# TencentYoutuResearch/NeRF-Loc

Measured on AMD Instinct MI355X. Metric: rendered rays/sec (4096 rays×128 samples, 256-wide MLP) at 1/2/4/8 MI355X, higher is better.
Workload: dtype f16mx (neural-point kernel, conv_out and feat_mlp.0: fp16 hi.hi + two MX-FP6 cross terms, 1.5 MFMA-equivalents per product; every other GEMM 3-term split-bf16 or split-fp16; fp32 accumulate; meets 1e-4)

## Files before the change

### nerf_loc_amd/csrc/knn.hip

```cpp
#include "common.h"

namespace {

constexpr int GRID_BITS = 6;
constexpr int GRID_N = 1 << GRID_BITS;
constexpr int GRID_CELLS = GRID_N * GRID_N * GRID_N;

__device__ __forceinline__ unsigned part1by2(unsigned x) {
  x &= 0x3ffu;
  x = (x | (x << 16)) & 0x030000FFu;
  x = (x | (x << 8)) & 0x0300F00Fu;
  x = (x | (x << 4)) & 0x030C30C3u;
  x = (x | (x << 2)) & 0x09249249u;
  return x;
}
__device__ __forceinline__ unsigned morton3(unsigned x, unsigned y, unsigned z) {
  return part1by2(x) | (part1by2(y) << 1) | (part1by2(z) << 2);
}

__global__ void knn_bbox_kernel(const float* __restrict__ xyz, int M, NlGridParams* gp) {
  __shared__ float smin[3][256], smax[3][256];
  float mn[3] = {3.4e38f, 3.4e38f, 3.4e38f}, mx[3] = {-3.4e38f, -3.4e38f, -3.4e38f};
  for (int i = threadIdx.x; i < M; i += blockDim.x) {
#pragma unroll
    for (int d = 0; d < 3; ++d) {
      float v = xyz[3 * (size_t)i + d];
      mn[d] = fminf(mn[d], v);
      mx[d] = fmaxf(mx[d], v);
    }
  }
#pragma unroll
  for (int d = 0; d < 3; ++d) { smin[d][threadIdx.x] = mn[d]; smax[d][threadIdx.x] = mx[d]; }
  __syncthreads();
  for (int s = blockDim.x / 2; s > 0; s >>= 1) {
    if ((int)threadIdx.x < s) {
#pragma unroll
      for (int d = 0; d < 3; ++d) {
        smin[d][threadIdx.x] = fminf(smin[d][threadIdx.x], smin[d][threadIdx.x + s]);
        smax[d][threadIdx.x] = fmaxf(smax[d][threadIdx.x], smax[d][threadIdx.x + s]);
      }
    }
    __syncthreads();
  }
  if (threadIdx.x == 0) {
    float ext = 0.f;
    for (int d = 0; d < 3; ++d) ext = fmaxf(ext, smax[d][0] - smin[d][0]);
    float cell = ext > 0.f ? ext / (float)GRID_N : 1.f;
    cell *= 1.0001f;
    gp->cell = cell;
    gp->inv_cell = 1.f / cell;
    for (int d = 0; d < 3; ++d) {
      gp->origin[d] = smin[d][0];
      gp->bmax[d] = smax[d][0];
      gp->dims[d] = GRID_N;
    }
    gp->ncells = GRID_CELLS;
  }
}

__device__ __forceinline__ int cell_coord(float v, float origin, float inv_cell) {
  int c = (int)floorf((v - origin) * inv_cell);
  return c < 0 ? 0 : (c >= GRID_N ? GRID_N - 1 : c);
}

__global__ void knn_count_kernel(const float* __restrict__ xyz, int M, const NlGridParams* __restrict__ gp,
                                 int* __restrict__ counts, int* __restrict__ cell_of) {
  int i = blockIdx.x * blockDim.x + threadIdx.x;
  if (i >= M) return;
  int cx = cell_coord(xyz[3 * (size_t)i + 0], gp->origin[0], gp->inv_cell);
  int cy = cell_coord(xyz[3 * (size_t)i + 1], gp->origin[1], gp->inv_cell);
  int cz = cell_coord(xyz[3 * (size_t)i + 2], gp->origin[2], gp->inv_cell);
  int cid = (int)morton3(cx, cy, cz);
  cell_of[i] = cid;
  atomicAdd(&counts[cid], 1);
}

__global__ void knn_scan_kernel(const int* __restrict__ counts, int* __restrict__ starts, int* __restrict__ cursor) {
  __shared__ int part[1024];
  const int n = GRID_CELLS;
  const int per = n / 1024;
  const int b = threadIdx.x * per;
  int s = 0;
  for (int i = b; i < b + per; ++i) s += counts[i];
  part[threadIdx.x] = s;
  __syncthreads();
  for (int o = 1; o < 1024; o <<= 1) {
    int v = (int)threadIdx.x >= o ? part[threadIdx.x - o] : 0;
    __syncthreads();
    part[threadIdx.x] += v;
    __syncthreads();
  }
  int run = threadIdx.x ? part[threadIdx.x - 1] : 0;
  for (int i = b; i < b + per; ++i) {
    starts[i] = run;
    cursor[i] = run;
    run += counts[i];
  }
  if (threadIdx.x == 1023) starts[n] = part[1023];
}

__global__ void knn_scatter_kernel(const float* __restrict__ xyz, int M, const int* __restrict__ cell_of,
                                   int* __restrict__ cursor, float4* __restrict__ sorted) {
  int i = blockIdx.x * blockDim.x + threadIdx.x;
  if (i >= M) return;
  int pos = atomicAdd(&cursor[cell_of[i]], 1);
  sorted[pos] = make_float4(xyz[3 * (size_t)i], xyz[3 * (size_t)i + 1], xyz[3 * (size_t)i + 2], __int_as_float(i));
}

typedef unsigned long long u64;

template <int CTRL, int ROWMASK>
__device__ __forceinline__ unsigned dpp_umin(unsigned v) {
  const unsigned t = (unsigned)__builtin_amdgcn_update_dpp((int)0xffffffffu, (int)v, CTRL, ROWMASK, 0xf, false);
  return t < v ? t : v;
}
__device__ __forceinline__ unsigned wave_umin(unsigned v) {
  v = dpp_umin<0x111, 0xf>(v);
  v = dpp_umin<0x112, 0xf>(v);
  v = dpp_umin<0x114, 0xf>(v);
  v = dpp_umin<0x118, 0xf>(v);
  v = dpp_umin<0x142, 0xa>(v);
  v = dpp_umin<0x143, 0xc>(v);
  return (unsigned)__builtin_amdgcn_readlane((int)v, 63);
}

template <int CTRL, int ROWMASK>
__device__ __forceinline__ unsigned dpp_umax(unsigned v) {
  const unsigned t = (unsigned)__builtin_amdgcn_update_dpp(0, (int)v, CTRL, ROWMASK, 0xf, false);
  return t > v ? t : v;
}
__device__ __forceinline__ unsigned wave_umax(unsigned v) {
  v = dpp_umax<0x111, 0xf>(v); v = dpp_umax<0x112, 0xf>(v); v = dpp_umax<0x114, 0xf>(v); v = dpp_umax<0x118, 0xf>(v);
  v = dpp_umax<0x142, 0xa>(v); v = dpp_umax<0x143, 0xc>(v);
  return (unsigned)__builtin_amdgcn_readlane((int)v, 63);
}

template <int K>
struct BestK {
  unsigned d, i, p;
  unsigned td, ti;
  __device__ __forceinline__ void clear() { d = i = td = ti = 0xffffffffu; p = 0; }
  __device__ __forceinline__ bool full() const { return ti != 0xffffffffu; }
  __device__ __forceinline__ void insert(unsigned nd, unsigned ni, unsigned np) {
    const unsigned pd = (unsigned)__builtin_amdgcn_update_dpp(0, (int)d, 0x111, 0xf, 0xf, false);
    const unsigned pi = (unsigned)__builtin_amdgcn_update_dpp(0, (int)i, 0x111, 0xf, 0xf, false);
    const unsigned pp = (unsigned)__builtin_amdgcn_update_dpp(0, (int)p, 0x111, 0xf, 0xf, false);
    const bool lt_me = nd < d || (nd == d && ni < i);
    const bool lt_prev = nd < pd || (nd == pd && ni < pi);
    d = lt_me ? (lt_prev ? pd : nd) : d;
    i = lt_me ? (lt_prev ? pi : ni) : i;
    p = lt_me ? (lt_prev ? pp : np) : p;
    td = (unsigned)__builtin_amdgcn_readlane((int)d, K - 1);
    ti = (unsigned)__builtin_amdgcn_readlane((int)i, K - 1);
  }
  __device__ __forceinline__ unsigned idx_at(int k) const { return (unsigned)__builtin_amdgcn_readlane((int)i, k); }
};

#ifdef KNN_STATS
__device__ unsigned long long knn_stats[16];
#define KNN_CNT(i, v) do { if (__lane_id() == 0) atomicAdd(&knn_stats[i], (unsigned long long)(v)); } while (0)
#else
#define KNN_CNT(i, v)
#endif
template <int K>
__device__ __forceinline__ void select_into(BestK<K>& best, unsigned kd, unsigned ki, unsigned kp) {
  while (true) {
    const bool cont = kd < best.td || (kd == best.td && ki < best.ti);
    if (__ballot(cont) == 0ull) break;
    KNN_CNT(2, 1);
    const unsigned dmin = wave_umin(cont ? kd : 0xffffffffu);
    const bool tie = cont && kd == dmin;
    const u64 tm = __ballot(tie);
    unsigned imin;
    int src = __builtin_ctzll(tm);
    if (__popcll(tm) == 1) imin = (unsigned)__builtin_amdgcn_readlane((int)ki, src);
    else {
      imin = wave_umin(tie ? ki : 0xffffffffu);
      src = __builtin_ctzll(__ballot(tie && ki == imin));
    }
    best.insert(dmin, imin, (unsigned)__builtin_amdgcn_readlane((int)kp, src));
    if (tie && ki == imin) { kd = 0xffffffffu; ki = 0xffffffffu; }
  }
}

struct QueryCtx {
  float qx, qy, qz, org0, org1, org2, cell, slack;
};

__device__ __forceinline__ float node_mindist2(const QueryCtx& c, unsigned cx, unsigned cy, unsigned cz, int L) {
  const float cl = c.cell * (float)(1 << L);
  const float x0 = c.org0 + (float)cx * cl, y0 = c.org1 + (float)cy * cl, z0 = c.org2 + (float)cz * cl;
  const float dx = fmaxf(fmaxf(x0 - c.qx, c.qx - (x0 + cl)) - c.slack, 0.f);
  const float dy = fmaxf(fmaxf(y0 - c.qy, c.qy - (y0 + cl)) - c.slack, 0.f);
  const float dz = fmaxf(fmaxf(z0 - c.qz, c.qz - (z0 + cl)) - c.slack, 0.f);
  return dx * dx + dy * dy + dz * dz;
}

template <int K, bool DEDUPE>
__device__ __forceinline__ void candidate(const QueryCtx& c, const float4* __restrict__ sorted, bool valid, int pos, const BestK<K>& best,
                                          unsigned& kd, unsigned& ki, bool dedupe_now = true, unsigned ubits = 0xffffffffu) {
  kd = 0xffffffffu; ki = 0xffffffffu;
  if (valid) {
    const float4 p = sorted[pos];
    const float ddx = c.qx - p.x, ddy = c.qy - p.y, ddz = c.qz - p.z;
    float d = __fmul_rn(ddx, ddx);
    d = __fadd_rn(d, __fmul_rn(ddy, ddy));
    d = __fadd_rn(d, __fmul_rn(ddz, ddz));
    kd = __float_as_uint(d);
    ki = (unsigned)__float_as_int(p.w);
    if (kd > ubits) { kd = 0xffffffffu; ki = 0xffffffffu; }
    if (DEDUPE && dedupe_now) {
      bool dup = false;
#pragma unroll
      for (int k = 0; k < K; ++k) dup |= (ki == best.idx_at(k));
      if (dup) { kd = 0xffffffffu; ki = 0xffffffffu; }
    }
  }
}

template <int K, bool DEDUPE, class Sink>
__device__ __forceinline__ void scan_range(const QueryCtx& c, const float4* __restrict__ sorted, int rs, int len, int lane, BestK<K>& best, Sink&& sink,
                                           bool dedupe_now = true, unsigned ubits = 0xffffffffu) {
  for (int base = 0; base < len; base += 64) {
    KNN_CNT(3, 1);
    unsigned kd, ki;
    candidate<K, DEDUPE>(c, sorted, base + lane < len, rs + base + lane, best, kd, ki, dedupe_now, ubits);
    sink(kd, ki, (unsigned)(rs + base + lane));
  }
}

constexpr int FRONT_CAP = 128;
constexpr int LEAF_CAP = 128;
constexpr int LEAF_COUNT_MAX = 8;

template <int K, int SPW>
__global__ __launch_bounds__(256) void knn_wave_kernel(const float* __restrict__ q, int N, const NlGridParams* __restrict__ gpp,
                                                       const int* __restrict__ starts, const float4* __restrict__ sorted,
                                                       int Kout, int* __restrict__ idx_out, float* __restrict__ d2_out) {
  __shared__ unsigned s_front[4][2][FRONT_CAP], s_fxyz[4][2][FRONT_CAP];
  __shared__ int s_leaf_s[4][LEAF_CAP], s_leaf_l[4][LEAF_CAP];
  __shared__ u64 s_ckey[4][64];
  __shared__ unsigned s_cpos[4][64];
  const int lane = threadIdx.x & 63, wv = threadIdx.x >> 6;
  const int n0 = __builtin_amdgcn_readfirstlane((nl_xcd_block() * 4 + wv) * SPW);
  QueryCtx c;
  c.org0 = gpp->origin[0]; c.org1 = gpp->origin[1]; c.org2 = gpp->origin[2];
  c.cell = gpp->cell; c.slack = 1e-3f * c.cell;
  const float inv_cell = gpp->inv_cell;
  bool prev_full = false;
  unsigned ppos = 0;
  bool pkeep = false;
  u64* const ckey = s_ckey[wv];
  unsigned* const cpos = s_cpos[wv];

  for (int sq = 0; sq < SPW; ++sq) {
  const int n = n0 + sq;
  if (n >= N) return;
  c.qx = q[3 * (size_t)n]; c.qy = q[3 * (size_t)n + 1]; c.qz = q[3 * (size_t)n + 2];

  BestK<K> best;
  best.clear();
  float U;
  const bool dedupe_now = !prev_full;
  bool deferred = prev_full;
  int ncand = 0;
  auto lds_list_handover = [&]() __attribute__((always_inline)) {
    __builtin_amdgcn_fence(__ATOMIC_RELEASE, "wavefront");
    __builtin_amdgcn_wave_barrier();
    __builtin_amdgcn_fence(__ATOMIC_ACQUIRE, "wavefront");
  };
  auto pour = [&]() __attribute__((always_inline)) {
    unsigned kd = 0xffffffffu, ki = 0xffffffffu, kp = 0;
    lds_list_handover();
    if (lane < ncand) { const u64 k = ckey[lane]; kd = (unsigned)(k >> 32); ki = (unsigned)k; kp = cpos[lane]; }
    select_into<K>(best, kd, ki, kp);
    ncand = 0;
    deferred = false;
  };
  const u64 lt_mask = (1ull << lane) - 1ull;
  auto sink = [&](unsigned kd, unsigned ki, unsigned kp) __attribute__((always_inline)) {
    if (!deferred) { select_into<K>(best, kd, ki, kp); return; }
    const bool v = ki != 0xffffffffu;
    const u64 mv = __ballot(v);
    if (mv == 0ull) return;
    const int cn = __popcll(mv);
    if (ncand + cn > 64) { pour(); select_into<K>(best, kd, ki, kp); return; }
    if (v) { const int pos = ncand + __popcll(mv & lt_mask); ckey[pos] = ((u64)kd << 32) | (u64)ki; cpos[pos] = kp; }
    ncand += cn;
  };
  if (!prev_full) {
    unsigned m = 0, mx = 0, my = 0, mz = 0;
    int L = GRID_BITS;
    while (L > 0) {
      unsigned key = 0xffffffffu;
      if (lane < 8) {
        const unsigned mc = (m << 3) | (unsigned)lane;
        const int sh = 3 * (L - 1);
        const int cnt = starts[(mc + 1) << sh] - starts[mc << sh];
        if (cnt >= K)
          key = (__float_as_uint(node_mindist2(c, 2 * mx + (lane & 1), 2 * my + ((lane >> 1) & 1), 2 * mz + ((lane >> 2) & 1), L - 1)) & ~7u) | (unsigned)lane;
      }
      key = wave_umin(key);
      if (key == 0xffffffffu) break;
      const unsigned ch = key & 7u;
      m = (m << 3) | ch;
      mx = 2 * mx + (ch & 1); my = 2 * my + ((ch >> 1) & 1); mz = 2 * mz + ((ch >> 2) & 1);
      --L;
    }
    const int rs0 = starts[m << (3 * L)], len0 = starts[(m + 1) << (3 * L)] - rs0;
    scan_range<K, false>(c, sorted, rs0, len0, lane, best, sink);
    U = best.full() ? __uint_as_float(best.td) : 3.4e38f;
  } else {
    float dprev = 0.f;
    if (pkeep) {
      const float4 pt = sorted[ppos];
      const float ddx = c.qx - pt.x, ddy = c.qy - pt.y, ddz = c.qz - pt.z;
      dprev = __fadd_rn(__fadd_rn(__fmul_rn(ddx, ddx), __fmul_rn(ddy, ddy)), __fmul_rn(ddz, ddz));
    }
    U = __uint_as_float(wave_umax(__float_as_uint(dprev)));
  }

  unsigned* front = s_front[wv][0];
  unsigned* nextf = s_front[wv][1];
  unsigned* fxyz = s_fxyz[wv][0];
  unsigned* nextx = s_fxyz[wv][1];
  int* leaf_s = s_leaf_s[wv];
  int* leaf_l = s_leaf_l[wv];
  int nfront = 1, nleaf = 0;
  int Lstart = GRID_BITS;
  if (U < 3.0e38f) {
    const float r = sqrtf(U * 1.000001f) + c.slack;
    const int lo0 = min(max((int)floorf((c.qx - r - c.org0) * inv_cell) - 1, 0), GRID_N - 1), hi0 = min(max((int)floorf((c.qx + r - c.org0) * inv_cell) + 1, 0), GRID_N - 1);
    const int lo1 = min(max((int)floorf((c.qy - r - c.org1) * inv_cell) - 1, 0), GRID_N - 1), hi1 = min(max((int)floorf((c.qy + r - c.org1) * inv_cell) + 1, 0), GRID_N - 1);
    const int lo2 = min(max((int)floorf((c.qz - r - c.org2) * inv_cell) - 1, 0), GRID_N - 1), hi2 = min(max((int)floorf((c.qz + r - c.org2) * inv_cell) + 1, 0), GRID_N - 1);
    int Ls = 1;
    while (Ls < GRID_BITS && (((hi0 >> Ls) - (lo0 >> Ls)) > 1 || ((hi1 >> Ls) - (lo1 >> Ls)) > 1 || ((hi2 >> Ls) - (lo2 >> Ls)) > 1)) ++Ls;
    Ls = __builtin_amdgcn_readfirstlane(Ls);
    if (Ls < GRID_BITS) {
      Lstart = Ls;
      const unsigned nx = (unsigned)(lo0 >> Ls) + (lane & 1), ny = (unsigned)(lo1 >> Ls) + ((lane >> 1) & 1), nz = (unsigned)(lo2 >> Ls) + ((lane >> 2) & 1);
      const bool ok = lane < 8 && nx <= (unsigned)(hi0 >> Ls) && ny <= (unsigned)(hi1 >> Ls) && nz <= (unsigned)(hi2 >> Ls);
      const u64 mk = __ballot(ok);
      if (ok) { const int pos = __popcll(mk & lt_mask); front[pos] = morton3(nx, ny, nz); fxyz[pos] = nx | (ny << 10) | (nz << 20); }
      nfront = __popcll(mk);
    }
  }
  if (Lstart == GRID_BITS && lane == 0) { front[0] = 0u; fxyz[0] = 0u; }
  KNN_CNT(4, Lstart); KNN_CNT(5, prev_full ? 0 : 1); KNN_CNT(6 + Lstart, 1);

  auto flush_leaves = [&]() {
    constexpr int SL = LEAF_COUNT_MAX;
    for (int b = 0; b < nleaf; b += 64 / SL) {
      KNN_CNT(1, 1);
      const int e = b + lane / SL;
      const bool ok = e < nleaf;
      const int rs = ok ? leaf_s[e] : 0, ln = ok ? leaf_l[e] : 0;
      unsigned kd, ki;
      candidate<K, true>(c, sorted, (lane % SL) < ln, rs + (lane % SL), best, kd, ki, dedupe_now, __float_as_uint(U));
      sink(kd, ki, (unsigned)(rs + (lane % SL)));
    }
    nleaf = 0;
    if (best.full()) U = fminf(U, __uint_as_float(best.td));
  };

  for (int L = Lstart; L > 0; --L) {
    int nnext = 0;
    const int sh = 3 * (L - 1);
    for (int base = 0; base < nfront; base += 8) {
      KNN_CNT(0, 1);
      const int ni = base + (lane >> 3);
      bool keep = false, leaf = false;
      unsigned mc = 0, cxyz = 0;
      int rs = 0, cnt = 0;
      if (ni < nfront) {
        mc = (front[ni] << 3) | (unsigned)(lane & 7);
        const unsigned pxyz = fxyz[ni];
        const unsigned cx = 2 * (pxyz & 1023u) + (lane & 1), cy = 2 * ((pxyz >> 10) & 1023u) + ((lane >> 1) & 1), cz = 2 * (pxyz >> 20) + ((lane >> 2) & 1);
        cxyz = cx | (cy << 10) | (cz << 20);
        rs = starts[mc << sh];
        cnt = starts[(mc + 1) << sh] - rs;
        keep = cnt > 0 && node_mindist2(c, cx, cy, cz, L - 1) <= U * 1.000001f;
        leaf = keep && (L - 1 == 0 || cnt <= LEAF_COUNT_MAX);
      }
      const bool inner = keep && !leaf;
      const u64 mi = __ballot(inner);
      const int ci = __popcll(mi);
      const int room = FRONT_CAP - nnext;
      const int pi = __popcll(mi & lt_mask);
      const bool spill = inner && pi >= room;
      if (inner && !spill) { nextf[nnext + pi] = mc; nextx[nnext + pi] = cxyz; }
      nnext += ci < room ? ci : room;
      const bool lf = leaf || spill;
      u64 mbig = __ballot(lf && cnt > LEAF_COUNT_MAX);
      while (mbig) {
        const int src = __builtin_ctzll(mbig);
        mbig &= mbig - 1;
        scan_range<K, true>(c, sorted, __builtin_amdgcn_readlane(rs, src), __builtin_amdgcn_readlane(cnt, src), lane, best, sink, dedupe_now, __float_as_uint(U));
        if (best.full()) U = fminf(U, __uint_as_float(best.td));
      }
      const bool small = lf && cnt <= LEAF_COUNT_MAX;
      const u64 ml = __ballot(small);
      const int cl_ = __popcll(ml);
      if (nleaf + cl_ > LEAF_CAP) flush_leaves();
      if (small) { const int p = nleaf + __popcll(ml & lt_mask); leaf_s[p] = rs; leaf_l[p] = cnt; }
      nleaf += cl_;
      if (nleaf >= 32) flush_leaves();
    }
    unsigned* t = front; front = nextf; nextf = t;
    t = fxyz; fxyz = nextx; nextx = t;
    nfront = nnext;
    if (nfront == 0) break;
  }
  if (nleaf > 0) flush_leaves();

  if (deferred && ncand < K) pour();
  if (deferred) {
    lds_list_handover();
    const u64 mine = lane < ncand ? ckey[lane] : ~0ull;
    const unsigned mlo = (unsigned)mine, mhi = (unsigned)(mine >> 32);
    int rank = 0;
    for (int jj = 0; jj < ncand; ++jj) {
      const u64 kj = ((u64)(unsigned)__builtin_amdgcn_readlane((int)mhi, jj) << 32) | (u64)(unsigned)__builtin_amdgcn_readlane((int)mlo, jj);
      rank += kj < mine ? 1 : 0;
    }
    const bool win = lane < ncand && rank < K;
    if (win && rank < Kout) {
      idx_out[(size_t)n * Kout + rank] = (int)mlo;
      d2_out[(size_t)n * Kout + rank] = __uint_as_float(mhi);
    }
    prev_full = true;
    pkeep = win;
    ppos = cpos[lane];
  } else {
    if (lane < Kout && lane < K) {
      const unsigned bd = best.d, bi = best.i;
      const bool ok = bi != 0xffffffffu;
      idx_out[(size_t)n * Kout + lane] = ok ? (int)bi : 0;
      d2_out[(size_t)n * Kout + lane] = ok ? __uint_as_float(bd) : 0.f;
    }
    prev_full = best.full();
    pkeep = lane < K;
    ppos = best.p;
  }
  }
}

}

size_t nl_knn_grid_bytes(int64_t M) {
  size_t b = 0;
  b += nl_align_up(sizeof(NlGridParams), 256);
  b += nl_align_up(sizeof(int) * (GRID_CELLS + 1), 256);
  b += 2 * nl_align_up(sizeof(int) * GRID_CELLS, 256);
  b += nl_align_up(sizeof(int) * (size_t)(M > 0 ? M : 1), 256);
  b += nl_align_up(sizeof(float4) * (size_t)(M > 0 ? M : 1), 256);
  return b;
}

int nl_knn_grid_build(NlKnnGrid* g, void* mem, const float* xyz, int64_t M, hipStream_t st) {
  char* p = (char*)mem;
  g->params = (NlGridParams*)p; p += nl_align_up(sizeof(NlGridParams), 256);
  g->starts = (int*)p; p += nl_align_up(sizeof(int) * (GRID_CELLS + 1), 256);
  g->counts = (int*)p; p += nl_align_up(sizeof(int) * GRID_CELLS, 256);
  g->cursor = (int*)p; p += nl_align_up(sizeof(int) * GRID_CELLS, 256);
  g->cell_of = (int*)p; p += nl_align_up(sizeof(int) * (size_t)(M > 0 ? M : 1), 256);
  g->sorted = (float4*)p;
  g->M = (int)M;
  if (M <= 0) return NL_OK;
  NL_CHECK_HIP(hipMemsetAsync(g->counts, 0, sizeof(int) * GRID_CELLS, st));
  hipLaunchKernelGGL(knn_bbox_kernel, dim3(1), dim3(256), 0, st, xyz, (int)M, g->params);
  int nb = (int)nl_cdiv(M, 256);
  hipLaunchKernelGGL(knn_count_kernel, dim3(nb), dim3(256), 0, st, xyz, (int)M, g->params, g->counts, g->cell_of);
  hipLaunchKernelGGL(knn_scan_kernel, dim3(1), dim3(1024), 0, st, g->counts, g->starts, g->cursor);
  hipLaunchKernelGGL(knn_scatter_kernel, dim3(nb), dim3(256), 0, st, xyz, (int)M, g->cell_of, g->cursor, g->sorted);
  NL_LAUNCH_CHECK();
  return NL_OK;
}

int nl_knn_search(const NlKnnGrid* g, const float* xyz, int64_t N, int K, int* idx, float* d2, hipStream_t st) {
  if (N <= 0) return NL_OK;
  if (g->M <= 0) {
    NL_CHECK_HIP(hipMemsetAsync(idx, 0, sizeof(int) * (size_t)N * K, st));
    NL_CHECK_HIP(hipMemsetAsync(d2, 0, sizeof(float) * (size_t)N * K, st));
    return NL_OK;
  }
  if (K < 1 || K > 8) return NL_ERR_UNSUPPORTED;
  constexpr int spw_small = 4;
  const bool big = N >= (1 << 18);
  const int spw = big ? 16 : spw_small;
  dim3 grid(nl_xcd_grid(nl_cdiv(N, 4 * spw)));
#define NL_KNN(KK, SPW) hipLaunchKernelGGL((knn_wave_kernel<KK, SPW>), grid, dim3(256), 0, st, xyz, (int)N, g->params, g->starts, g->sorted, K, idx, d2)
  if (K == 1) { if (big) NL_KNN(1, 16); else NL_KNN(1, spw_small); }
  else { if (big) NL_KNN(8, 16); else NL_KNN(8, spw_small); }
#undef NL_KNN
  NL_LAUNCH_CHECK();
#ifdef KNN_STATS
  {
    unsigned long long h[16];
    hipStreamSynchronize(st);
    hipMemcpyFromSymbol(h, HIP_SYMBOL(knn_stats), sizeof(h));
    fprintf(stderr, "knn stats per query (N = %lld): frontier batches %.2f, leaf batches %.2f, selection iterations %.2f, range batches %.2f, start level %.2f, phase-1 %.3f; start-level histogram",
            (long long)N, (double)h[0] / N, (double)h[1] / N, (double)h[2] / N, (double)h[3] / N, (double)h[4] / N, (double)h[5] / N);
    for (int l = 0; l <= GRID_BITS; ++l) fprintf(stderr, " %d:%.3f", l, (double)h[6 + l] / N);
    fprintf(stderr, "\n");
    hipMemset(nullptr, 0, 0);
    unsigned long long z[16] = {0};
    hipMemcpyToSymbol(HIP_SYMBOL(knn_stats), z, sizeof(z));
  }
#endif
  return NL_OK;
}
```

### nerf_loc_amd/csrc/mvdec.h

```cpp
#pragma once
#include "common.h"
#include "mfma.h"

namespace nlmv {

struct Taps {
  int x0, y0;
  float nw, ne, sw, se;
  bool mw, me, mn, ms;
};

template <bool ALIGN, bool BORDER>
__device__ __forceinline__ Taps make_taps(float xn, float yn, int Wm, int Hm) {
  float ix, iy;
  if (ALIGN) {
    ix = (xn + 1.f) * ((float)(Wm - 1) / 2.f);
    iy = (yn + 1.f) * ((float)(Hm - 1) / 2.f);
  } else {
    ix = (xn + 1.f) * ((float)Wm / 2.f) - 0.5f;
    iy = (yn + 1.f) * ((float)Hm / 2.f) - 0.5f;
  }
  if (BORDER) {
    ix = fminf((float)(Wm - 1), fmaxf(ix, 0.f));
    iy = fminf((float)(Hm - 1), fmaxf(iy, 0.f));
  }
  float xw = floorf(ix), yn0 = floorf(iy);
  float w = ix - xw, e = 1.f - w, n = iy - yn0, s = 1.f - n;
  Taps t;
  t.nw = s * e; t.ne = s * w; t.sw = n * e; t.se = n * w;
  xw = fminf(fmaxf(xw, -2.f), (float)Wm + 1.f);
  yn0 = fminf(fmaxf(yn0, -2.f), (float)Hm + 1.f);
  t.x0 = (int)xw; t.y0 = (int)yn0;
  t.mw = t.x0 >= 0 && t.x0 < Wm;
  t.me = t.x0 + 1 >= 0 && t.x0 + 1 < Wm;
  t.mn = t.y0 >= 0 && t.y0 < Hm;
  t.ms = t.y0 + 1 >= 0 && t.y0 + 1 < Hm;
  return t;
}

__device__ __forceinline__ unsigned pack_taps(const Taps& t, int w, int h) {
  const int x0 = min(max(t.x0, 0), w - 1), x1 = min(max(t.x0 + 1, 0), w - 1);
  const int y0 = min(max(t.y0, 0), h - 1), y1 = min(max(t.y0 + 1, 0), h - 1);
  return (unsigned)(y0 * w + x0) | ((unsigned)(x1 - x0) << 30) | ((unsigned)(y1 - y0) << 31);
}
__device__ __forceinline__ void unpack_taps(unsigned pk, int w, int (&o)[4]) {
  const int base = (int)(pk & 0x3fffffffu), dx = (int)((pk >> 30) & 1u), dy = (pk >> 31) ? w : 0;
  o[0] = base; o[1] = base + dx; o[2] = base + dy; o[3] = base + dy + dx;
}


constexpr int DEC_STRIDE = 1024 + 32 + 1024 + 32 + 64 + 2;

__device__ __forceinline__ void decoder(const float* __restrict__ w, const float (&x)[32], float& o0, float& o1) {
  float h1[32], h2[32];
#pragma unroll
  for (int j = 0; j < 32; ++j) {
    float a = w[1024 + j];
#pragma unroll
    for (int i = 0; i < 32; ++i) a = fmaf(w[j * 32 + i], x[i], a);
    h1[j] = nl_elu(a);
  }
  const float* w2 = w + 1024 + 32;
#pragma unroll
  for (int j = 0; j < 32; ++j) {
    float a = w2[1024 + j];
#pragma unroll
    for (int i = 0; i < 32; ++i) a = fmaf(w2[j * 32 + i], h1[i], a);
    h2[j] = nl_elu(a);
  }
  const float* w4 = w2 + 1024 + 32;
  float a0 = w4[64], a1 = w4[65];
#pragma unroll
  for (int i = 0; i < 32; ++i) {
    a0 = fmaf(w4[i], h2[i], a0);
    a1 = fmaf(w4[32 + i], h2[i], a1);
  }
  o0 = a0;
  o1 = a1;
}


__device__ __forceinline__ bool project_neuray(const float* P, float X, float Y, float Z, int Wimg, int H, float& px, float& py, float& depth) {
  const float cx = fmaf(P[2], Z, fmaf(P[1], Y, P[0] * X)) + P[3];
  const float cy = fmaf(P[6], Z, fmaf(P[5], Y, P[4] * X)) + P[7];
  depth = fmaf(P[10], Z, fmaf(P[9], Y, P[8] * X)) + P[11];
  const bool bad = fabsf(depth) < 1e-4f;
  if (bad) depth = 1e-3f;
  px = cx / depth; py = cy / depth;
  const bool outside = (px < -0.5f) | (px >= (float)Wimg - 0.5f) | (py < -0.5f) | (py >= (float)H - 0.5f);
  return !bad && !outside;
}

__device__ __forceinline__ void sample_visf(const float* __restrict__ base, int h, int w, int Wimg, int H, float px, float py, bool valid, float (&x)[32]) {
  if (valid) {
    const float xn = px / (float)(Wimg - 1) * 2.f - 1.f;
    const float yn = py / (float)(H - 1) * 2.f - 1.f;
    const Taps t = make_taps<false, true>(xn, yn, w, h);
    const int xe = t.x0 + 1, ys = t.y0 + 1;
#pragma unroll
    for (int c4 = 0; c4 < 8; ++c4) {
      float4 a = make_float4(0, 0, 0, 0), b = a, c = a, d = a;
      if (t.mn && t.mw) a = *(const float4*)(base + ((size_t)t.y0 * w + t.x0) * 32 + c4 * 4);
      if (t.mn && t.me) b = *(const float4*)(base + ((size_t)t.y0 * w + xe) * 32 + c4 * 4);
      if (t.ms && t.mw) c = *(const float4*)(base + ((size_t)ys * w + t.x0) * 32 + c4 * 4);
      if (t.ms && t.me) d = *(const float4*)(base + ((size_t)ys * w + xe) * 32 + c4 * 4);
      x[c4 * 4 + 0] = a.x * t.nw + b.x * t.ne + c.x * t.sw + d.x * t.se;
      x[c4 * 4 + 1] = a.y * t.nw + b.y * t.ne + c.y * t.sw + d.y * t.se;
      x[c4 * 4 + 2] = a.z * t.nw + b.z * t.ne + c.z * t.sw + d.z * t.se;
      x[c4 * 4 + 3] = a.w * t.nw + b.w * t.ne + c.w * t.sw + d.w * t.se;
    }
  } else {
#pragma unroll
    for (int i = 0; i < 32; ++i) x[i] = 0.f;
  }
}

__device__ __forceinline__ void decode_all(const float* __restrict__ dw, const float (&x)[32], float& m0, float& m1, float& v0, float& v1, float& vs, float& aw) {
  float dummy;
  decoder(dw + 0 * DEC_STRIDE, x, m0, m1);
  decoder(dw + 1 * DEC_STRIDE, x, v0, v1);
  decoder(dw + 2 * DEC_STRIDE, x, aw, dummy);
  decoder(dw + 3 * DEC_STRIDE, x, vs, dummy);
  m0 = nl_softplus(m0); m1 = nl_softplus(m1);
  v0 = nl_softplus(v0) + 0.05f; v1 = nl_softplus(v1) + 0.05f;
  aw = nl_sigmoid(aw); vs = nl_sigmoid(vs);
}


constexpr int MVD_W1 = 0;
constexpr int MVD_W2 = 1024;
constexpr int MVD_F32 = 2048;
constexpr int MVD_NF32 = (128 + 128 + 256 + 8) / 4;
constexpr int MVD_F16 = MVD_F32 + MVD_NF32;
constexpr int MVD_T = MVD_F16 + 2048;
constexpr int MVD_PACK_UINT4 = MVD_T + 2048;
constexpr int MVD_LDS_UINT4 = 2048 + MVD_NF32;

template <bool X3>
__device__ __forceinline__ void mvd_load_lds(uint4* sw, const uint4* __restrict__ dpack, int tid, int nthreads) {
  for (int i = tid; i < 2048; i += nthreads) sw[i] = dpack[(X3 ? MVD_F16 : 0) + i];
  for (int i = tid; i < MVD_NF32; i += nthreads) sw[2048 + i] = dpack[MVD_F32 + i];
}

template <bool X3> struct MvdOps;
template <> struct MvdOps<true> {
  typedef nl_f16x8 v8;
  static __device__ __forceinline__ void split(const float (&v)[8], v8& hi, v8& lo) {
    nl_u32x4 h, l;
#pragma unroll
    for (int t = 0; t < 4; ++t) {
      unsigned hp, lp; float l0, l1;
      asm("v_cvt_pk_f16_f32 %0, %3, %4\n\tv_fma_mix_f32 %1, %0, -1.0, %3 op_sel_hi:[1,0,0]\n\tv_fma_mix_f32 %2, %0, -1.0, %4 op_sel:[1,0,0] op_sel_hi:[1,0,0]"
          : "=&v"(hp), "=&v"(l0), "=&v"(l1) : "v"(v[2 * t]), "v"(v[2 * t + 1]));
      asm("v_cvt_pk_f16_f32 %0, %1, %2" : "=v"(lp) : "v"(l0), "v"(l1));
      h[t] = hp; l[t] = lp;
    }
    hi = __builtin_bit_cast(v8, h); lo = __builtin_bit_cast(v8, l);
  }
  static __device__ __forceinline__ nl_f32x16 mfma(v8 a, v8 b, nl_f32x16 c) { return __builtin_amdgcn_mfma_f32_32x32x16_f16(a, b, c, 0, 0, 0); }
};
template <> struct MvdOps<false> {
  typedef nl_bf16x8 v8;
  static __device__ __forceinline__ void split(const float (&v)[8], v8& hi, v8& lo) {
#pragma unroll
    for (int t = 0; t < 8; ++t) hi[t] = (__bf16)v[t];
    lo = hi;
  }
  static __device__ __forceinline__ nl_f32x16 mfma(v8 a, v8 b, nl_f32x16 c) { return __builtin_amdgcn_mfma_f32_32x32x16_bf16(a, b, c, 0, 0, 0); }
};

__device__ __forceinline__ void mvd_elu2(float& a, float& b) { const nl_f32x2 e = nl_elu_fast2(nl_f32x2{a, b}); a = e[0]; b = e[1]; }

__device__ __forceinline__ void mvd_tap16(const float* __restrict__ base , int vh, int vw_, int Wimg, int H, float px, float py,
                                          bool valid, float (&x0)[8], float (&x1)[8]) {
  const float xn = px / (float)(Wimg - 1) * 2.f - 1.f;
  const float yn = py / (float)(H - 1) * 2.f - 1.f;
  const Taps t = make_taps<false, true>(xn, yn, vw_, vh);
  const size_t o00 = ((size_t)(t.mn ? t.y0 : 0) * vw_ + (t.mw ? t.x0 : 0)) * 32;
  const size_t o01 = ((size_t)(t.mn ? t.y0 : 0) * vw_ + (t.me ? t.x0 + 1 : 0)) * 32;
  const size_t o10 = ((size_t)(t.ms ? t.y0 + 1 : 0) * vw_ + (t.mw ? t.x0 : 0)) * 32;
  const size_t o11 = ((size_t)(t.ms ? t.y0 + 1 : 0) * vw_ + (t.me ? t.x0 + 1 : 0)) * 32;
  const float w00 = (valid && t.mn && t.mw) ? t.nw : 0.f, w01 = (valid && t.mn && t.me) ? t.ne : 0.f;
  const float w10 = (valid && t.ms && t.mw) ? t.sw : 0.f, w11 = (valid && t.ms && t.me) ? t.se : 0.f;
#pragma unroll
  for (int g = 0; g < 2; ++g) {
#pragma unroll
    for (int c4 = 0; c4 < 2; ++c4) {
      const int co = 16 * g + 4 * c4;
      const float4 a = *(const float4*)(base + o00 + co), b = *(const float4*)(base + o01 + co);
      const float4 c = *(const float4*)(base + o10 + co), d = *(const float4*)(base + o11 + co);
      float* dst = g ? x1 : x0;
      dst[4 * c4 + 0] = fmaf(d.x, w11, fmaf(c.x, w10, fmaf(b.x, w01, a.x * w00)));
      dst[4 * c4 + 1] = fmaf(d.y, w11, fmaf(c.y, w10, fmaf(b.y, w01, a.y * w00)));
      dst[4 * c4 + 2] = fmaf(d.z, w11, fmaf(c.z, w10, fmaf(b.z, w01, a.z * w00)));
      dst[4 * c4 + 3] = fmaf(d.w, w11, fmaf(c.w, w10, fmaf(b.w, w01, a.w * w00)));
    }
  }
}

template <bool X3>
__device__ __forceinline__ void mvd_decode_tile(const uint4* sw, int lane, const float (&x0)[8], const float (&x1)[8], float& m0, float& m1,
                                                float& v0, float& v1, float& vs, float& aw) {
  typedef MvdOps<X3> OP;
  typedef typename OP::v8 v8;
  const int hh = lane >> 5;
  const float* sf = reinterpret_cast<const float*>(sw + 2048);
  const float* b1 = sf, *b2 = sf + 128, *w4p = sf + 256, *b4 = sf + 512;
  v8 xh[2], xl[2];
  OP::split(x0, xh[0], xl[0]);
  OP::split(x1, xh[1], xl[1]);
  float o[4][2];
#pragma unroll
  for (int d = 0; d < 4; ++d) {
    nl_f32x16 acc;
#pragma unroll
    for (int g = 0; g < 4; ++g) {
      const float4 b = *(const float4*)(b1 + 32 * d + 8 * g + 4 * hh);
      acc[4 * g] = b.x; acc[4 * g + 1] = b.y; acc[4 * g + 2] = b.z; acc[4 * g + 3] = b.w;
    }
#pragma unroll
    for (int q = 0; q < 2; ++q) {
      const v8 ah = __builtin_bit_cast(v8, sw[MVD_W1 + (q * 4 + d) * 64 + lane]);
      if (X3) {
        const v8 al = __builtin_bit_cast(v8, sw[MVD_W1 + 512 + (q * 4 + d) * 64 + lane]);
        acc = OP::mfma(al, xh[q], acc);
        acc = OP::mfma(ah, xl[q], acc);
      }
      acc = OP::mfma(ah, xh[q], acc);
    }
    v8 gh[2], gl[2];
#pragma unroll
    for (int s = 0; s < 2; ++s) {
      float vv[8];
#pragma unroll
      for (int t = 0; t < 8; ++t) vv[t] = acc[8 * s + t];
#pragma unroll
      for (int t = 0; t < 8; t += 2) mvd_elu2(vv[t], vv[t + 1]);
      OP::split(vv, gh[s], gl[s]);
    }
    nl_f32x16 acc2;
#pragma unroll
    for (int g = 0; g < 4; ++g) {
      const float4 b = *(const float4*)(b2 + 32 * d + 8 * g + 4 * hh);
      acc2[4 * g] = b.x; acc2[4 * g + 1] = b.y; acc2[4 * g + 2] = b.z; acc2[4 * g + 3] = b.w;
    }
#pragma unroll
    for (int s = 0; s < 2; ++s) {
      const v8 ah = __builtin_bit_cast(v8, sw[MVD_W2 + (d * 2 + s) * 64 + lane]);
      if (X3) {
        const v8 al = __builtin_bit_cast(v8, sw[MVD_W2 + 512 + (d * 2 + s) * 64 + lane]);
        acc2 = OP::mfma(al, gh[s], acc2);
        acc2 = OP::mfma(ah, gl[s], acc2);
      }
      acc2 = OP::mfma(ah, gh[s], acc2);
    }
    float h2[16];
#pragma unroll
    for (int r = 0; r < 16; ++r) h2[r] = acc2[r];
#pragma unroll
    for (int r = 0; r < 16; r += 2) mvd_elu2(h2[r], h2[r + 1]);
#pragma unroll
    for (int u = 0; u < 2; ++u) {
      float p = 0.f;
      if (u == 0 || d < 2) {
        const float* w = w4p + ((d * 2 + u) * 2 + hh) * 16;
#pragma unroll
        for (int r4 = 0; r4 < 4; ++r4) {
          const float4 ww = *(const float4*)(w + 4 * r4);
          p = fmaf(ww.x, h2[4 * r4], p); p = fmaf(ww.y, h2[4 * r4 + 1], p);
          p = fmaf(ww.z, h2[4 * r4 + 2], p); p = fmaf(ww.w, h2[4 * r4 + 3], p);
        }
        p += __shfl_xor(p, 32, 64);
        p += b4[d * 2 + u];
      }
      o[d][u] = p;
    }
  }
  m0 = nl_softplus(o[0][0]); m1 = nl_softplus(o[0][1]);
  v0 = nl_softplus(o[1][0]) + 0.05f; v1 = nl_softplus(o[1][1]) + 0.05f;
  aw = nl_sigmoid(o[2][0]); vs = nl_sigmoid(o[3][0]);
}

}
```

Baseline: 580,100.

## Streamline KNN octree descent arithmetic and merge fp16 split asm

After: 584,900, median of 6. Within noise of the previous version (+0.8%).

```diff
diff --git a/nerf_loc_amd/csrc/knn.hip b/nerf_loc_amd/csrc/knn.hip
--- a/nerf_loc_amd/csrc/knn.hip
+++ b/nerf_loc_amd/csrc/knn.hip
@@ -108,6 +108,16 @@
 }
 
 typedef unsigned long long u64;
+
+__device__ __forceinline__ unsigned dilate6(unsigned x) {
+  x = (x | (x << 8)) & 0x300Fu;
+  x = (x | (x << 4)) & 0x30C3u;
+  x = (x | (x << 2)) & 0x9249u;
+  return x;
+}
+__device__ __forceinline__ int lanes_below(u64 m) {
+  return (int)__builtin_amdgcn_mbcnt_hi((unsigned)(m >> 32), __builtin_amdgcn_mbcnt_lo((unsigned)m, 0u));
+}
 
 template <int CTRL, int ROWMASK>
 __device__ __forceinline__ unsigned dpp_umin(unsigned v) {
@@ -184,16 +194,19 @@
 }
 
 struct QueryCtx {
-  float qx, qy, qz, org0, org1, org2, cell, slack;
+  float qx, qy, qz, cell, slack;
+  float ax, ay, az;
 };
 
-__device__ __forceinline__ float node_mindist2(const QueryCtx& c, unsigned cx, unsigned cy, unsigned cz, int L) {
-  const float cl = c.cell * (float)(1 << L);
-  const float x0 = c.org0 + (float)cx * cl, y0 = c.org1 + (float)cy * cl, z0 = c.org2 + (float)cz * cl;
-  const float dx = fmaxf(fmaxf(x0 - c.qx, c.qx - (x0 + cl)) - c.slack, 0.f);
-  const float dy = fmaxf(fmaxf(y0 - c.qy, c.qy - (y0 + cl)) - c.slack, 0.f);
-  const float dz = fmaxf(fmaxf(z0 - c.qz, c.qz - (z0 + cl)) - c.slack, 0.f);
-  return dx * dx + dy * dy + dz * dz;
+struct LevelBox {
+  float cl, nw;
+  __device__ __forceinline__ LevelBox(const QueryCtx& c, int L) : cl(c.cell * (float)(1 << L)), nw(-(cl + 4.f * c.slack)) {}
+};
+
+__device__ __forceinline__ float node_mindist2(const QueryCtx& c, const LevelBox& b, unsigned cxyz) {
+  const float lx = fmaf((float)(cxyz & 255u), b.cl, c.ax), ly = fmaf((float)((cxyz >> 8) & 255u), b.cl, c.ay), lz = fmaf((float)((cxyz >> 16) & 255u), b.cl, c.az);
+  const float dx = fmaxf(fmaxf(lx, b.nw - lx), 0.f), dy = fmaxf(fmaxf(ly, b.nw - ly), 0.f), dz = fmaxf(fmaxf(lz, b.nw - lz), 0.f);
+  return fmaf(dz, dz, fmaf(dy, dy, dx * dx));
 }
 
 template <int K, bool DEDUPE>
@@ -244,9 +257,12 @@
   const int lane = threadIdx.x & 63, wv = threadIdx.x >> 6;
   const int n0 = __builtin_amdgcn_readfirstlane((nl_xcd_block() * 4 + wv) * SPW);
   QueryCtx c;
-  c.org0 = gpp->origin[0]; c.org1 = gpp->origin[1]; c.org2 = gpp->origin[2];
   c.cell = gpp->cell; c.slack = 1e-3f * c.cell;
+  const float wo0 = gpp->origin[0] - 2.f * c.slack, wo1 = gpp->origin[1] - 2.f * c.slack, wo2 = gpp->origin[2] - 2.f * c.slack;
   const float inv_cell = gpp->inv_cell;
+  const unsigned lane_xyz = (unsigned)((lane & 1) | ((lane & 2) << 7) | ((lane & 4) << 14));
+  const int sl_axis = min(lane >> 4, 2), sl_level = ((lane & 15) >> 1) + 1;
+  const float sl_org = gpp->origin[sl_axis], sl_sign = (lane & 1) ? 1.f : -1.f;
   bool prev_full = false;
   unsigned ppos = 0;
   bool pkeep = false;
@@ -257,6 +273,8 @@
   const int n = n0 + sq;
   if (n >= N) return;
   c.qx = q[3 * (size_t)n]; c.qy = q[3 * (size_t)n + 1]; c.qz = q[3 * (size_t)n + 2];
+  c.ax = wo0 - c.qx; c.ay = wo1 - c.qy; c.az = wo2 - c.qz;
+  const float sl_q = q[3 * (size_t)n + sl_axis];
 
   BestK<K> best;
   best.clear();
@@ -277,7 +295,6 @@
     ncand = 0;
     deferred = false;
   };
-  const u64 lt_mask = (1ull << lane) - 1ull;
   auto sink = [&](unsigned kd, unsigned ki, unsigned kp) __attribute__((always_inline)) {
     if (!deferred) { select_into<K>(best, kd, ki, kp); return; }
     const bool v = ki != 0xffffffffu;
@@ -285,11 +302,11 @@
     if (mv == 0ull) return;
     const int cn = __popcll(mv);
     if (ncand + cn > 64) { pour(); select_into<K>(best, kd, ki, kp); return; }
-    if (v) { const int pos = ncand + __popcll(mv & lt_mask); ckey[pos] = ((u64)kd << 32) | (u64)ki; cpos[pos] = kp; }
+    if (v) { const int pos = ncand + lanes_below(mv); ckey[pos] = ((u64)kd << 32) | (u64)ki; cpos[pos] = kp; }
     ncand += cn;
   };
   if (!prev_full) {
-    unsigned m = 0, mx = 0, my = 0, mz = 0;
+    unsigned m = 0, mxyz = 0;
     int L = GRID_BITS;
     while (L > 0) {
       unsigned key = 0xffffffffu;
@@ -297,14 +314,13 @@
         const unsigned mc = (m << 3) | (unsigned)lane;
         const int sh = 3 * (L - 1);
         const int cnt = starts[(mc + 1) << sh] - starts[mc << sh];
-        if (cnt >= K)
-          key = (__float_as_uint(node_mindist2(c, 2 * mx + (lane & 1), 2 * my + ((lane >> 1) & 1), 2 * mz + ((lane >> 2) & 1), L - 1)) & ~7u) | (unsigned)lane;
+        if (cnt >= K) key = (__float_as_uint(node_mindist2(c, LevelBox(c, L - 1), (mxyz << 1) | lane_xyz)) & ~7u) | (unsigned)lane;
       }
       key = wave_umin(key);
       if (key == 0xffffffffu) break;
       const unsigned ch = key & 7u;
       m = (m << 3) | ch;
-      mx = 2 * mx + (ch & 1); my = 2 * my + ((ch >> 1) & 1); mz = 2 * mz + ((ch >> 2) & 1);
+      mxyz = (mxyz << 1) | (ch & 1) | ((ch & 2) << 7) | ((ch & 4) << 14);
       --L;
     }
     const int rs0 = starts[m << (3 * L)], len0 = starts[(m + 1) << (3 * L)] - rs0;
@@ -329,20 +345,28 @@
   int nfront = 1, nleaf = 0;
   int Lstart = GRID_BITS;
   if (U < 3.0e38f) {
-    const float r = sqrtf(U * 1.000001f) + c.slack;
-    const int lo0 = min(max((int)floorf((c.qx - r - c.org0) * inv_cell) - 1, 0), GRID_N - 1), hi0 = min(max((int)floorf((c.qx + r - c.org0) * inv_cell) + 1, 0), GRID_N - 1);
-    const int lo1 = min(max((int)floorf((c.qy - r - c.org1) * inv_cell) - 1, 0), GRID_N - 1), hi1 = min(max((int)floorf((c.qy + r - c.org1) * inv_cell) + 1, 0), GRID_N - 1);
-    const int lo2 = min(max((int)floorf((c.qz - r - c.org2) * inv_cell) - 1, 0), GRID_N - 1), hi2 = min(max((int)floorf((c.qz + r - c.org2) * inv_cell) + 1, 0), GRID_N - 1);
-    int Ls = 1;
-    while (Ls < GRID_BITS && (((hi0 >> Ls) - (lo0 >> Ls)) > 1 || ((hi1 >> Ls) - (lo1 >> Ls)) > 1 || ((hi2 >> Ls) - (lo2 >> Ls)) > 1)) ++Ls;
-    Ls = __builtin_amdgcn_readfirstlane(Ls);
+    const float r = __builtin_amdgcn_sqrtf(fmaxf(U * 1.000001f, 1.17549435e-38f)) * 1.000001f + c.slack;
+    const int end = min(max((int)floorf(((sl_q + sl_sign * r) - sl_org) * inv_cell) + ((lane & 1) ? 1 : -1), 0), GRID_N - 1);
+    const int hi = __builtin_amdgcn_update_dpp(0, end, 0xB1 , 0xf, 0xf, false);
+    const u64 fine = __ballot(((hi >> sl_level) - (end >> sl_level)) > 1) & 0x0000015501550155ull;
+    const unsigned fl = (unsigned)(fine | (fine >> 16) | (fine >> 32)) & 0x155u;
+    const int Ls = fl ? ((31 - __builtin_clz(fl)) >> 1) + 2 : 1;
     if (Ls < GRID_BITS) {
       Lstart = Ls;
-      const unsigned nx = (unsigned)(lo0 >> Ls) + (lane & 1), ny = (unsigned)(lo1 >> Ls) + ((lane >> 1) & 1), nz = (unsigned)(lo2 >> Ls) + ((lane >> 2) & 1);
-      const bool ok = lane < 8 && nx <= (unsigned)(hi0 >> Ls) && ny <= (unsigned)(hi1 >> Ls) && nz <= (unsigned)(hi2 >> Ls);
-      const u64 mk = __ballot(ok);
-      if (ok) { const int pos = __popcll(mk & lt_mask); front[pos] = morton3(nx, ny, nz); fxyz[pos] = nx | (ny << 10) | (nz << 20); }
-      nfront = __popcll(mk);
+      const unsigned nd = (unsigned)(end >> Ls);
+      const unsigned w = dilate6(nd) | (nd << 16);
+      const unsigned x0 = (unsigned)__builtin_amdgcn_readlane((int)w, 0), x1 = (unsigned)__builtin_amdgcn_readlane((int)w, 1);
+      const unsigned y0 = (unsigned)__builtin_amdgcn_readlane((int)w, 16), y1 = (unsigned)__builtin_amdgcn_readlane((int)w, 17);
+      const unsigned z0 = (unsigned)__builtin_amdgcn_readlane((int)w, 32), z1 = (unsigned)__builtin_amdgcn_readlane((int)w, 33);
+      const unsigned mk = (x1 != x0 ? 0xffu : 0x55u) & (y1 != y0 ? 0xffu : 0x33u) & (z1 != z0 ? 0xffu : 0x0fu);
+      const unsigned cx0 = x0 & 0xffffu, cx1 = x1 & 0xffffu, cy0 = (y0 & 0xffffu) << 1, cy1 = (y1 & 0xffffu) << 1, cz0 = (z0 & 0xffffu) << 2, cz1 = (z1 & 0xffffu) << 2;
+      const unsigned c000 = cx0 | cy0 | cz0;
+      if (lane < 8 && ((mk >> lane) & 1u)) {
+        const int pos = lanes_below((u64)mk);
+        front[pos] = c000 ^ (-(lane & 1) & (cx0 ^ cx1)) ^ (-((lane >> 1) & 1) & (cy0 ^ cy1)) ^ (-((lane >> 2) & 1) & (cz0 ^ cz1));
+        fxyz[pos] = ((x0 >> 16) | ((y0 >> 16) << 8) | ((z0 >> 16) << 16)) + lane_xyz;
+      }
+      nfront = __popc(mk);
     }
   }
   if (Lstart == GRID_BITS && lane == 0) { front[0] = 0u; fxyz[0] = 0u; }
@@ -365,7 +389,10 @@
 
   for (int L = Lstart; L > 0; --L) {
     int nnext = 0;
-    const int sh = 3 * (L - 1);
+    const int sh2 = 3 * (L - 1) + 2;
+    const char* const starts_lo = (const char*)starts;
+    const char* const starts_hi = (const char*)(starts + (1 << (sh2 - 2)));
+    const LevelBox box(c, L - 1);
     for (int base = 0; base < nfront; base += 8) {
       KNN_CNT(0, 1);
       const int ni = base + (lane >> 3);
@@ -374,19 +401,18 @@
       int rs = 0, cnt = 0;
       if (ni < nfront) {
         mc = (front[ni] << 3) | (unsigned)(lane & 7);
-        const unsigned pxyz = fxyz[ni];
-        const unsigned cx = 2 * (pxyz & 1023u) + (lane & 1), cy = 2 * ((pxyz >> 10) & 1023u) + ((lane >> 1) & 1), cz = 2 * (pxyz >> 20) + ((lane >> 2) & 1);
-        cxyz = cx | (cy << 10) | (cz << 20);
-        rs = starts[mc << sh];
-        cnt = starts[(mc + 1) << sh] - rs;
-        keep = cnt > 0 && node_mindist2(c, cx, cy, cz, L - 1) <= U * 1.000001f;
+        cxyz = (fxyz[ni] << 1) | lane_xyz;
+        const unsigned off = mc << sh2;
+        rs = *(const int*)(starts_lo + off);
+        cnt = *(const int*)(starts_hi + off) - rs;
+        keep = cnt > 0 && node_mindist2(c, box, cxyz) <= U * 1.000001f;
         leaf = keep && (L - 1 == 0 || cnt <= LEAF_COUNT_MAX);
       }
       const bool inner = keep && !leaf;
       const u64 mi = __ballot(inner);
       const int ci = __popcll(mi);
       const int room = FRONT_CAP - nnext;
-      const int pi = __popcll(mi & lt_mask);
+      const int pi = lanes_below(mi);
       const bool spill = inner && pi >= room;
       if (inner && !spill) { nextf[nnext + pi] = mc; nextx[nnext + pi] = cxyz; }
       nnext += ci < room ? ci : room;
@@ -402,7 +428,7 @@
       const u64 ml = __ballot(small);
       const int cl_ = __popcll(ml);
       if (nleaf + cl_ > LEAF_CAP) flush_leaves();
-      if (small) { const int p = nleaf + __popcll(ml & lt_mask); leaf_s[p] = rs; leaf_l[p] = cnt; }
+      if (small) { const int p = nleaf + lanes_below(ml); leaf_s[p] = rs; leaf_l[p] = cnt; }
       nleaf += cl_;
       if (nleaf >= 32) flush_leaves();
     }
diff --git a/nerf_loc_amd/csrc/mvdec.h b/nerf_loc_amd/csrc/mvdec.h
--- a/nerf_loc_amd/csrc/mvdec.h
+++ b/nerf_loc_amd/csrc/mvdec.h
@@ -146,15 +146,15 @@
 template <> struct MvdOps<true> {
   typedef nl_f16x8 v8;
   static __device__ __forceinline__ void split(const float (&v)[8], v8& hi, v8& lo) {
-    nl_u32x4 h, l;
-#pragma unroll
-    for (int t = 0; t < 4; ++t) {
-      unsigned hp, lp; float l0, l1;
-      asm("v_cvt_pk_f16_f32 %0, %3, %4\n\tv_fma_mix_f32 %1, %0, -1.0, %3 op_sel_hi:[1,0,0]\n\tv_fma_mix_f32 %2, %0, -1.0, %4 op_sel:[1,0,0] op_sel_hi:[1,0,0]"
-          : "=&v"(hp), "=&v"(l0), "=&v"(l1) : "v"(v[2 * t]), "v"(v[2 * t + 1]));
-      asm("v_cvt_pk_f16_f32 %0, %1, %2" : "=v"(lp) : "v"(l0), "v"(l1));
-      h[t] = hp; l[t] = lp;
-    }
+    nl_u32x4 h, l; float t;
+#define MVD_SPLIT_PAIR(H, L, A, B) \
+    "v_cvt_pk_f16_f32 " H ", " A ", " B "\n\tv_fma_mix_f32 " L ", " H ", -1.0, " A " op_sel_hi:[1,0,0]\n\tv_fma_mix_f32 %8, " H ", -1.0, " B " op_sel:[1,0,0] op_sel_hi:[1,0,0]\n\t" \
+    "v_cvt_pk_f16_f32 " L ", " L ", %8"
+    asm(MVD_SPLIT_PAIR("%0", "%4", "%9", "%10") "\n\t" MVD_SPLIT_PAIR("%1", "%5", "%11", "%12") "\n\t" MVD_SPLIT_PAIR("%2", "%6", "%13", "%14") "\n\t"
+        MVD_SPLIT_PAIR("%3", "%7", "%15", "%16")
+        : "=&v"(h[0]), "=&v"(h[1]), "=&v"(h[2]), "=&v"(h[3]), "=&v"(l[0]), "=&v"(l[1]), "=&v"(l[2]), "=&v"(l[3]), "=&v"(t)
+        : "v"(v[0]), "v"(v[1]), "v"(v[2]), "v"(v[3]), "v"(v[4]), "v"(v[5]), "v"(v[6]), "v"(v[7]));
+#undef MVD_SPLIT_PAIR
     hi = __builtin_bit_cast(v8, h); lo = __builtin_bit_cast(v8, l);
   }
   static __device__ __forceinline__ nl_f32x16 mfma(v8 a, v8 b, nl_f32x16 c) { return __builtin_amdgcn_mfma_f32_32x32x16_f16(a, b, c, 0, 0, 0); }
```
